# Nextomics/NextDenovo

Measured on AMD Instinct MI355X. Metric: corrected bases/sec, higher is better.
Workload: dtype int32

## Files before the change

### include/ndgpu_nextcorrect.h

```cpp
#ifndef NDGPU_NEXTCORRECT_H
#define NDGPU_NEXTCORRECT_H

#include <stdint.h>

#ifdef __cplusplus
extern "C" {
#endif
#pragma GCC visibility push(default)

typedef struct {
    unsigned int len;
    float identity;
    char *seq;
} consensus_trimed;

consensus_trimed *nextCorrect(char **seqs, unsigned int *aln_start, unsigned int *aln_end, unsigned int seq_count,
                              unsigned int max_mem_len, unsigned int min_len_aln, unsigned int max_cov_aln,
                              unsigned int min_cov, unsigned int lqseq_max_length, float min_error_corrected_ratio,
                              unsigned int split, unsigned int fast, int read_type);

void free_consensus_trimed(consensus_trimed *c);

typedef struct {
    unsigned int shift;
// ... 158 lines not shown
    uint64_t poa_resident_jobs;
    uint64_t poa_resident_declined;
    uint64_t poa_graph_launches;
    double poa_graph_ms;
    uint64_t poa_h2d_bytes;
    uint64_t poa_d2h_bytes;
    uint64_t cns_jobs;
    uint64_t cns_declined;
    uint64_t cns_launches;
    uint64_t cns_regions;
    double cns_ms;
    uint64_t cns_d2h_bytes;
    uint64_t walk_d2h_bytes;
} ndgpu_stats;
void ndgpu_get_stats(ndgpu_stats *out);
void ndgpu_reset_stats(void);
uint64_t ndgpu_release_memory(void);
void ndgpu_reserve_device_memory(uint64_t bytes);
int ndgpu_device_count(void);

#pragma GCC visibility pop
#ifdef __cplusplus
}
#endif
#endif
```

### nextdenovo_amd/api.py

```python
from __future__ import annotations

import ctypes as C
import os

os.environ.setdefault("GPU_MAX_HW_QUEUES", "16")

from . import build as _build

_LIB = None
_BIG = C.c_char * (1 << 30)


class ConsensusTrimed(C.Structure):
    _fields_ = [("len", C.c_uint), ("identity", C.c_float), ("seq", C.c_void_p)]


class PoaJob(C.Structure):
    _fields_ = [("seqs", C.POINTER(C.c_char_p)), ("len", C.POINTER(C.c_uint16)), ("seq_count", C.c_int32)]


class RankJob(C.Structure):
    _fields_ = [("seqs", C.POINTER(C.c_char_p)), ("len", C.POINTER(C.c_uint16)), ("seq_count", C.c_int32)]


# ... 100 lines not shown
    lib.ndgpu_poa_batch.argtypes = [C.POINTER(PoaJob), C.c_int, C.POINTER(C.c_void_p)]
    lib.ndgpu_poa_batch.restype = C.c_int
    lib.ndgpu_poa_batch_flags.argtypes = [C.POINTER(PoaJob), C.c_int, C.c_int, C.POINTER(C.c_void_p)]
    lib.ndgpu_poa_batch_flags.restype = C.c_int
    lib.ndgpu_lq_rank_batch.argtypes = [C.POINTER(RankJob), C.c_int, C.c_int, C.POINTER(RankResult)]
    lib.ndgpu_lq_rank_batch.restype = C.c_int
    lib.ndgpu_cns_windows_batch.argtypes = [C.POINTER(CnsJob), C.c_int, C.c_int, C.POINTER(CnsResult), C.POINTER(C.c_void_p),
                                            C.POINTER(C.c_void_p)]
    lib.ndgpu_cns_windows_batch.restype = C.c_int
    lib.ndgpu_align_batch.argtypes = [C.POINTER(AlnJob), C.c_int, C.c_int, C.POINTER(AlnResult), C.POINTER(C.c_void_p),
                                      C.POINTER(C.c_void_p), C.POINTER(C.c_void_p)]
    lib.ndgpu_align_batch.restype = C.c_int
    lib.ndgpu_align_db_batch.argtypes = [C.c_void_p, C.POINTER(AlnDbJob)] + lib.ndgpu_align_batch.argtypes[1:]
    lib.ndgpu_align_db_batch.restype = C.c_int
    lib.ndgpu_get_stats.argtypes = [C.POINTER(Stats)]
    lib.ndgpu_reset_stats.argtypes = []
    lib.ndgpu_device_count.restype = C.c_int
    return lib


def _take(lib, r):
    ln = r.contents.len
    ide = r.contents.identity
    seq = C.string_at(r.contents.seq, ln) if ln > 4 else b""
    lib.free_consensus_trimed(r)
    return ln, ide, seq


def correct(seqs, aln_start, aln_end, max_aln_length, min_len_aln=500, max_cov_aln=130, min_cov_base=4,
            max_lq_length=10000, min_error_corrected_ratio=0.8, split=0, fast=0, read_type=1):
# ... 328 lines not shown


def stats() -> dict:
    lib = load()
    s = Stats()
    lib.ndgpu_get_stats(C.byref(s))
    names = [f[0] for f in Stats._fields_]
    late = [n for n in names if n in _POA_RESIDENT_STATS]
    names = [n for n in names if n not in _POA_RESIDENT_STATS]
    at = names.index("poa_ms") + 1
    names[at:at] = late
    late = [n for n in names if n in _CNS_STATS]
    names = [n for n in names if n not in _CNS_STATS]
    at = names.index("backtrack_ms") + 1
    names[at:at] = late
    return {n: getattr(s, n) for n in names}


def release_device_memory() -> int:
    lib = load()
    lib.ndgpu_release_memory.restype = C.c_uint64
    return int(lib.ndgpu_release_memory())


def reserve_device_memory(n_bytes: int):
    lib = load()
    lib.ndgpu_reserve_device_memory.argtypes = [C.c_uint64]
    lib.ndgpu_reserve_device_memory.restype = None
    lib.ndgpu_reserve_device_memory(int(max(0, n_bytes)))


# ... 7 lines not shown
```

### nextdenovo_amd/csrc/capi.cpp

```cpp
#include <hip/hip_runtime_api.h>
#include <cerrno>
#include <sys/uio.h>
#include <unistd.h>

#include <algorithm>
#include <atomic>
#include <cstdio>
#include <cstdlib>
#include <cstring>
#include <string>
#include <chrono>
#include <functional>
#include <mutex>
#include <thread>
#include <vector>

#include "../../include/ndgpu_nextcorrect.h"
#include "nd_host.h"
#include "nd_cns.h"
#include "nd_runtime.h"
#include "nd_subplan.h"

using namespace ndgpu;

// ... 1011 lines not shown
    o->lq_aln_columns = s.lq_aln_columns, o->lq_bases = s.lq_bases, o->lq_out = s.lq_out;
    o->lq_jobs = s.lq_jobs, o->lq_repairs = s.lq_repairs;
    o->tb_tasks = s.tb_tasks, o->tb_walkers = s.tb_walkers, o->tb_fallbacks = s.tb_fallbacks;
    o->poa_jobs = s.poa_jobs, o->poa_declined = s.poa_declined, o->poa_rounds = s.poa_rounds, o->poa_launches = s.poa_launches;
    o->poa_cells = s.poa_cells, o->poa_ms = s.poa_ms;
    o->rank_jobs = s.rank_jobs, o->rank_tail = s.rank_tail, o->rank_launches = s.rank_launches, o->rank_ms = s.rank_ms;
    o->aln_batch_jobs = s.aln_batch_jobs, o->aln_batch_launches = s.aln_batch_launches, o->aln_batch_runs = s.aln_batch_runs;
    o->aln_batch_ms = s.aln_batch_ms;
    o->poa_resident_jobs = s.poa_resident_jobs, o->poa_resident_declined = s.poa_resident_declined;
    o->poa_graph_launches = s.poa_graph_launches, o->poa_graph_ms = s.poa_graph_ms;
    o->poa_h2d_bytes = s.poa_h2d_bytes, o->poa_d2h_bytes = s.poa_d2h_bytes;
    o->cns_jobs = s.cns_jobs, o->cns_declined = s.cns_declined, o->cns_launches = s.cns_launches, o->cns_regions = s.cns_regions;
    o->cns_ms = s.cns_ms, o->cns_d2h_bytes = s.cns_d2h_bytes, o->walk_d2h_bytes = s.walk_d2h_bytes;
}

void ndgpu_reset_stats(void) { DeviceAligner::reset_all_stats(); }

uint64_t ndgpu_release_memory(void) {
    size_t f0 = 0, f1 = 0, t = 0;
    (void)hipMemGetInfo(&f0, &t);
    join_reapers();
    for (int c = 0; c < DeviceAligner::kMaxContexts; c++)
        if (DeviceAligner *d = DeviceAligner::peek(c)) (void)d->release_memory_if_idle();
    (void)hipMemGetInfo(&f1, &t);
    return f1 > f0 ? (uint64_t)(f1 - f0) : 0;
}

void ndgpu_reserve_device_memory(uint64_t bytes) { DeviceAligner::reserve_device_memory(bytes); }

int ndgpu_device_count(void) {
// ... 7 lines not shown
```

### nextdenovo_amd/csrc/device_runtime.hip

```cpp
#include <hip/hip_runtime.h>

#include <algorithm>
#include <string>
#include <atomic>
#include <cassert>
#include <chrono>
#include <cmath>
#include <cstdio>
#include <cstdlib>
#include <cstring>
#include <condition_variable>
#include <mutex>
#include <set>
#include <thread>
#include <type_traits>
#include <unordered_map>
#include <vector>

#include "nd_device.h"
#include "nd_host.h"
#include "nd_lqplan.h"
#include "nd_runtime.h"

namespace ndgpu {
// ... 241 lines not shown
    X(uint32_t, d_ops, device, levelled)                                                                                                  \
    X(AlnTask, d_tasks, device, levelled)                                                                                                 \
    X(AlnOut, d_outs, device, levelled)                                                                                                   \
    X(uint64_t, d_trace, device, levelled)                                                                                                \
    X(int32_t, d_v, device, levelled)                                                                                                     \
                                                                  \
    X(uint64_t, d_wtrace, device, levelled)                                                                                               \
    X(int32_t, d_wmink, device, levelled)                                                                                                 \
    X(AlnTask, d_wtasks, device, levelled)        \
       \
    X(uint32_t, d_ck_cells, device, levelled)                                                                                             \
    X(uint2, d_ck_hdr, device, levelled)                                                                                                  \
    X(TbSeg, d_tbseg, device, levelled)                                                                                                   \
    X(TbSegOut, d_tbout, device, levelled)                                                                                                \
    X(int32_t, d_ids, device, levelled)                                                                                                   \
         \
    X(AlnRunSum, d_run_sums, device, levelled)                                                                                            \
    X(uint32_t, d_run_skip, device, levelled)                                                                                             \
    X(uint64_t, d_run_off, device, levelled)                                                                                              \
    X(uint32_t, d_runs, device, levelled)                                                                                                 \
                                                                                       \
    X(ReadDev, d_reads, device, levelled)                                                                                                 \
    X(PileDev, d_piles, device, levelled)                                                                                                 \
    X(uint32_t, d_read_pile, device, levelled)                                                                                            \
    X(uint32_t, d_acc, device, levelled)                                                                                                  \
    X(uint32_t, d_tags, device, levelled)                                                                                                 \
    X(uint32_t, d_colidx, device, levelled)                                                                                               \
    X(uint32_t, d_cov, device, levelled)                        \
    X(uint32_t, d_cellbase, device, levelled)                                                                                             \
    X(uint32_t, d_entbase, device, levelled)                                                                                              \
// ... 240 lines not shown
        if (dst_host && bytes) pending.push_back(Pending{dst_host, down_used, bytes});
        down_used += need;
        return at;
    }

    struct Phase {
        std::unique_lock<std::mutex> dbg;
        std::lock_guard<std::mutex> lock;
        explicit Phase(State &S) : dbg(g_debug_exclusive ? std::unique_lock<std::mutex>(g_dbg_mu) : std::unique_lock<std::mutex>()), lock(S.mu) {
            HIP_CHECK(hipSetDevice(S.device));
        }
    };

    std::vector<AlignChunk> plan_chunks(AlnTask *t, size_t nt);
    void launch_chunk(const AlignChunk &c, const int32_t *order, const int32_t *tb_order, hipEvent_t ev_mid, hipEvent_t ev_end, const char *who);
    void tally_outs(size_t nt, std::vector<int32_t> *wide);
    void run_wide(bool ops_to_host, const std::vector<int32_t> &ids);

    MainLayout layout_piles(MainPile **mp, size_t np);
    void reserve_layout(const MainLayout &L, size_t np);
    const int32_t *length_order(size_t a, size_t m);
    void align_main(const std::vector<AlignChunk> &chunks, size_t np);
    void launch_tags(const CovPlanes &cov, size_t np);
    void upload_plan(const MsaPlan &plan);
    MsaResult count_and_score(const MsaPlan &plan, const CovPlanes &cov, const CnsPlan *cns);
    CnsPlan plan_cns(const MsaPlan &plan, MainPile **mp);
    void launch_cns(const CnsPlan &cns, const PileDev *dev_piles, const PathItem *dev_path);
    void fetch_cns(const CnsPlan &cns, const MsaResult &res, const std::vector<uint8_t> &bad_pile, MainPile **mp);
    void score_pass(const MsaPlan &plan, const K10Args &k10);
    void rescue_pass(const MsaPlan &plan, const K10Args &k10);
// ... 118 lines not shown
        t.links += s.links; t.score_launches += s.score_launches; t.backtrack_ms += s.backtrack_ms;
        t.score_segments += s.score_segments; t.score_repairs += s.score_repairs; t.score_slow_piles += s.score_slow_piles;
        t.traceback_launches += s.traceback_launches; t.lq_launches += s.lq_launches; t.lq_columns += s.lq_columns;
        t.lq_aln_columns += s.lq_aln_columns; t.lq_bases += s.lq_bases; t.lq_out += s.lq_out; t.lq_jobs += s.lq_jobs; t.lq_repairs += s.lq_repairs;
        t.tb_tasks += s.tb_tasks; t.tb_walkers += s.tb_walkers; t.tb_fallbacks += s.tb_fallbacks;
        t.poa_jobs += s.poa_jobs; t.poa_declined += s.poa_declined; t.poa_rounds += s.poa_rounds; t.poa_launches += s.poa_launches;
        t.poa_cells += s.poa_cells; t.poa_ms += s.poa_ms;
        t.poa_resident_jobs += s.poa_resident_jobs; t.poa_resident_declined += s.poa_resident_declined;
        t.poa_graph_launches += s.poa_graph_launches; t.poa_graph_ms += s.poa_graph_ms;
        t.poa_h2d_bytes += s.poa_h2d_bytes; t.poa_d2h_bytes += s.poa_d2h_bytes;
        t.rank_jobs += s.rank_jobs; t.rank_tail += s.rank_tail; t.rank_launches += s.rank_launches; t.rank_ms += s.rank_ms;
        t.aln_batch_jobs += s.aln_batch_jobs; t.aln_batch_launches += s.aln_batch_launches; t.aln_batch_runs += s.aln_batch_runs;
        t.aln_batch_ms += s.aln_batch_ms;
        t.cns_jobs += s.cns_jobs; t.cns_declined += s.cns_declined; t.cns_launches += s.cns_launches; t.cns_regions += s.cns_regions;
        t.cns_ms += s.cns_ms; t.cns_d2h_bytes += s.cns_d2h_bytes; t.walk_d2h_bytes += s.walk_d2h_bytes;
    }
    t.allocs = g_alloc_calls.load(), t.alloc_ms = (double)g_alloc_ns.load() * 1e-6;
    t.level_allocs = g_level_calls.load(), t.level_ms = (double)g_level_ns.load() * 1e-6;
    return t;
}

void DeviceAligner::reset_all_stats() {
    g_alloc_calls = 0, g_alloc_ns = 0, g_level_calls = 0, g_level_ns = 0;
    for (int i = 0; i < kMaxContexts; i++)
        if (DeviceAligner *c = peek(i)) c->reset_stats();
}

uint32_t *DeviceAligner::upload_db(const uint32_t *pool_words, size_t n_words, int device) {
    HIP_CHECK(hipSetDevice(device));
    uint32_t *d = nullptr;
// ... 246 lines not shown
    if (max_sg) {
        d_ck_cells.reserve(max_ck * kCkptCells + 1);
        d_ck_hdr.reserve(max_ck + 1);
        d_tbseg.reserve(max_sg);
        d_tbout.reserve(max_sg);
    }
    return chunks;
}

void DeviceAligner::State::launch_chunk(const AlignChunk &c, const int32_t *order, const int32_t *tb_order, hipEvent_t ev_mid,
                                        hipEvent_t ev_end, const char *who) {
    const AlnTask *tk = d_tasks.p + c.begin;
    AlnOut *out = d_outs.p + c.begin;
    const int n = (int)(c.end - c.begin);
    const TbArgs tb{d_ck_cells.p, d_ck_hdr.p, d_tbseg.p, d_tbout.p, (int)c.slots, hooks_of<TbConfig>().cshift, hooks_of<TbConfig>().warm};
    if (c.seg) launch_ond_forward_ckpt(tk, out, d_pool.p, db_pool, d_trace.p, d_ops.p, tb, n, stream, order);
    else launch_ond_forward(tk, out, d_pool.p, db_pool, d_trace.p, n, stream, order);
    HIP_CHECK(hipEventRecord(ev_mid, stream));
    if (who) NDGPU_DBG(stream, "%s: traceback", who);
    if (c.seg) launch_ond_traceback_seg(tk, out, d_pool.p, db_pool, d_trace.p, d_ops.p, tb, n, stream);
    else launch_ond_traceback(tk, out, d_pool.p, db_pool, d_trace.p, nullptr, d_ops.p, nullptr, n, stream, tb_order);
    if (ev_end) HIP_CHECK(hipEventRecord(ev_end, stream));
}

void DeviceAligner::State::tally_outs(size_t nt, std::vector<int32_t> *wide) {
    for (size_t i = 0; i < nt; i++) {
        const AlnOut &o = h_outs.p[i];
        stats.cells += (uint64_t)o.cells;
        stats.d_steps += (uint64_t)o.d_steps;
        stats.trace_words += (uint64_t)o.trace_end;
        if (o.fin_idx & kTbSeen) {
            stats.tb_tasks++;
            stats.tb_walkers += (uint64_t)(o.d_final > 0 ? (o.d_final - 1) >> hooks_of<TbConfig>().cshift : 0) + 1;
            if (o.fin_idx & kTbRefused) stats.tb_fallbacks++;
        }
        if ((uint32_t)o.max_band > stats.max_band) stats.max_band = (uint32_t)o.max_band;
        if (wide && o.status == ST_NEED_WIDE) wide->push_back((int32_t)i);
        if (o.status == ST_ALIGNED) {
            stats.trace_bits += (uint64_t)o.cells;
            stats.columns += (uint64_t)o.n_cols;
        }
    }
}

static size_t next_chunk(AlnJob *const *jobs, size_t n, uint64_t trace_budget_bytes) {
    static const size_t max_jobs = getenv("NDGPU_ALIGN_CHUNK_JOBS") ? (size_t)std::max(1ll, atoll(getenv("NDGPU_ALIGN_CHUNK_JOBS"))) : ~(size_t)0;
    size_t take = 0;
    uint64_t bytes = 0;
    while (take < n && take < max_jobs) {
        const AlnJob &j = *jobs[take];
        int md, bd;
        limits_for(j.q_len + j.t_len, j.hq, &md, &bd);
        const uint64_t b = task_trace_bytes(md);
        if (take && bytes + b > trace_budget_bytes) break;
        bytes += b;
        take++;
    }
// ... 77 lines not shown
    pool.insert(pool.end(), kPoolPadWords, 0u);

    S.d_pool.reserve(pool.size());
    S.d_tasks.reserve(n);
    S.d_outs.reserve(n);
    const std::vector<AlignChunk> chunks = S.plan_chunks(tasks.data(), n);
    assert(chunks.size() == 1);
    S.d_ops.reserve(ops_words + 2);
    if (ops_to_host) S.h_ops.reserve(ops_words + 2);
    S.h_outs.reserve(n);

    hipStream_t st = S.stream;
    const uint64_t tc1 = wall_ns();
    S.h2d(S.d_pool.p, pool.data(), pool.size() * sizeof(uint32_t), st);
    S.h2d(S.d_tasks.p, tasks.data(), n * sizeof(AlnTask), st);
    S.mark(State::kEvFrontK7, st);
    NDGPU_DBG(st, "chunk: forward %zu tasks", n);
    S.launch_chunk(chunks[0], nullptr, nullptr, S.evs[State::kEvFrontK8a], nullptr, "chunk");
    NDGPU_DBG(st, "chunk: done");
    HIP_CHECK(hipMemcpyAsync(S.h_outs.p, S.d_outs.p, n * sizeof(AlnOut), hipMemcpyDeviceToHost, st));
    if (ops_to_host) HIP_CHECK(hipMemcpyAsync(S.h_ops.p, S.d_ops.p, ops_words * sizeof(uint32_t), hipMemcpyDeviceToHost, st));
    S.sync_drain(st);
    HIP_CHECK(hipGetLastError());
    S.stats.forward_ms += S.ms(State::kEvFrontK7, State::kEvFrontK8a);
    S.stats.forward_launches++;
    S.stats.tasks += n;

    std::vector<int32_t> wide;
    for (size_t i = 0; i < n; i++)
        if (S.h_outs.p[i].status == ST_NEED_WIDE) wide.push_back((int32_t)i);
    if (!wide.empty()) S.run_wide(ops_to_host, wide);
    *dev_ns = wall_ns() - tc1;

    S.tally_outs(n, nullptr);
    if (std::find(bad.begin(), bad.end(), 1) != bad.end()) {
        static bool warned = false;
// ... 261 lines not shown
    d_lq_jobs.reserve(L.jobs.size() + 1), d_lq_hdr.reserve(L.hdr_words + 1);
    d_lq_lnk.reserve(L.lnk_words + 64);
    d_lq_out.reserve(L.out_bytes + 1), d_lq_tmp.reserve(L.cell_rows + 1), d_lq_bnd.reserve((L.jobs.size() + 1) * 4 * (size_t)kLqLinkCap);
    return plan_chunks(tasks.data(), nt);
}

std::vector<char> DeviceAligner::State::launch_lq(LqLayout &L, const std::vector<AlignChunk> &chunks) {
    hipStream_t st = stream;
    const size_t n = L.piles.size(), nt = tasks.size();
    h2d(d_pool.p, pool.data(), pool.size() * sizeof(uint32_t), st);
    h2d(d_tasks.p, tasks.data(), nt * sizeof(AlnTask), st);
    h2d(d_lq_piles.p, L.piles.data(), n * sizeof(LqPileDev), st);
    h2d(d_lq_pieces.p, L.pieces.data(), L.pieces.size() * sizeof(LqPieceDev), st);
    if (!L.jobs.empty()) h2d(d_lq_jobs.p, L.jobs.data(), L.jobs.size() * sizeof(LqJobDev), st);
    grow_lq_evs(2 * chunks.size() + 1);
    HIP_CHECK(hipEventRecord(lq_evs[0], st));
    for (size_t c = 0; c < chunks.size(); c++) {
        NDGPU_DBG(st, "lq: forward / traceback %zu..%zu of %zu tasks", chunks[c].begin, chunks[c].end, nt);
        launch_chunk(chunks[c], nullptr, nullptr, lq_evs[2 * c + 1], lq_evs[2 * c + 2], nullptr);
    }
    mark(kEvLqMsaBegin, st);
    NDGPU_DBG(st, "lq: msa of %zu piles", n);
    launch_lq_msa(d_lq_piles.p, d_lq_jobs.p, d_lq_pieces.p, d_tasks.p, d_outs.p, d_ops.p, d_pool.p, d_lq_hdr.p, d_lq_lnk.p, d_lq_rec.p,
                  d_lq_bnd.p, d_lq_tmp.p, d_lq_out.p, (int)n, (int)L.jobs.size(), hooks_of<LqHooks>().warm, hooks_of<LqHooks>().force_repair, st);
    mark(kEvLqMsaEnd, st);
    h_outs.reserve(nt + 1);
    HIP_CHECK(hipMemcpyAsync(h_outs.p, d_outs.p, nt * sizeof(AlnOut), hipMemcpyDeviceToHost, st));
    std::vector<char> out(L.out_bytes + 1);
    d2h(L.piles.data(), d_lq_piles.p, n * sizeof(LqPileDev), st);
    if (L.out_bytes) d2h(out.data(), d_lq_out.p, L.out_bytes, st);
    sync_drain(st);
    HIP_CHECK(hipGetLastError());
    return out;
}

void DeviceAligner::State::tally_lq(LqRound **rounds, const LqLayout &L, size_t n_chunks, const std::vector<char> &out) {
    const size_t nt = tasks.size();
    for (size_t c = 0; c < n_chunks; c++) {
        stats.forward_ms += ms_between(lq_evs[2 * c], lq_evs[2 * c + 1]);
        stats.traceback_ms += ms_between(lq_evs[2 * c + 1], lq_evs[2 * c + 2]);
    }
    stats.forward_launches += n_chunks, stats.traceback_launches += n_chunks;
// ... 154 lines not shown
    auto cls_of = [&](size_t i) {
        const uint32_t c = ((uint32_t)tasks[a + i].q_len + (uint32_t)tasks[a + i].t_len) >> 6;
        return (kLenClasses - 1) - std::min<uint32_t>(c, kLenClasses - 1);
    };
    for (size_t i = 0; i < m; i++) order_cls[cls_of(i) + 1]++;
    for (uint32_t c = 0; c < kLenClasses; c++) order_cls[c + 1] += order_cls[c];
    for (size_t i = 0; i < m; i++) order[order_cls[cls_of(i)]++] = (int32_t)i;
    d_ids.reserve(m);
    h2d(d_ids.p, order.data(), m * sizeof(int32_t), stream);
    return d_ids.p;
}

void DeviceAligner::State::align_main(const std::vector<AlignChunk> &chunks, size_t np) {
    hipStream_t st = stream;
    const size_t nt = tasks.size();
    for (const AlignChunk &ch : chunks) {
        NDGPU_DBG(st, "main: forward %zu..%zu of %zu tasks, %zu piles", ch.begin, ch.end, nt, np);
        const int32_t *ids = length_order(ch.begin, ch.end - ch.begin);
        mark(kEvMainK7, st);
        launch_chunk(ch, ids, hooks_of<MainHooks>().k8_order ? ids : nullptr, evs[kEvMainK8a], evs[kEvMainAligned], "main");
        NDGPU_DBG(st, "main: traceback done");
        HIP_CHECK(hipEventSynchronize(evs[kEvMainAligned]));
        stats.forward_ms += ms(kEvMainK7, kEvMainK8a);
        stats.forward_launches++;
        stats.traceback_ms += ms(kEvMainK8a, kEvMainAligned);
        stats.traceback_launches++;
    }
    if (!nt) return;
    HIP_CHECK(hipMemcpyAsync(h_outs.p, d_outs.p, nt * sizeof(AlnOut), hipMemcpyDeviceToHost, st));
    sync_drain(st);
    std::vector<int32_t> wide;
    tally_outs(nt, &wide);
    if (!wide.empty()) run_wide(false, wide);
    stats.tasks += nt;
}

void DeviceAligner::State::launch_tags(const CovPlanes &cov, size_t np) {
    hipStream_t st = stream;
    const int nr = (int)reads.size();
    mark(kEvTagsBegin, st);
    NDGPU_DBG(st, "main: shift_scan");
    launch_shift_scan(d_tasks.p, d_outs.p, d_ops.p, d_reads.p, nr, st);
    NDGPU_DBG(st, "main: pile_accept");
    launch_pile_accept(d_piles.p, d_reads.p, d_acc.p, cov.cov, (int)np, st);
// ... 974 lines not shown
```

### nextdenovo_amd/csrc/nd_device.h

```cpp
#pragma once

#include <cstdint>

#include "nd_lockstep.h"

namespace ndgpu {

struct AlnTask {
    uint64_t q_off;
    uint64_t t_off;
    int32_t q_len;
    int32_t t_len;
    int32_t max_d;
    int32_t band;
    uint64_t trace_off;
    uint64_t mink_off;
    uint64_t ops_off;
    uint32_t ops_cap;
    uint32_t row_words;
    uint64_t v_off;
    uint32_t v_mask;
    uint32_t seg_off;
};

// ... 46 lines not shown
constexpr int32_t kTbRefused = 1 << 16;
constexpr int32_t kTbSeen = 1 << 17;

constexpr uint32_t kTagHead = 0u;
__host__ __device__ inline uint32_t tag_pack(int32_t t_pos, uint32_t delta, uint32_t base) {
    return ((uint32_t)(t_pos + 1) << 11) | (delta << 3) | base;
}
__host__ __device__ inline int32_t tag_tpos(uint32_t g) { return (int32_t)(g >> 11) - 1; }
__host__ __device__ inline uint32_t tag_delta(uint32_t g) { return (g >> 3) & 0xffu; }
__host__ __device__ inline uint32_t tag_base(uint32_t g) { return g & 7u; }

#if defined(SIMT_EMULATION)
inline unsigned long long wave_ballot(bool p) { return __ballot(p); }
#elif defined(__HIPCC__)
__device__ __forceinline__ unsigned long long wave_ballot(bool p) { return __builtin_amdgcn_ballot_w64(p); }
#endif

struct ReadDev {
    int32_t task;
    uint32_t aln_start;
    uint32_t aln_end;
    uint64_t tag_off;
    uint64_t colidx_off;
    uint32_t shift;
    uint32_t aln_len;
    uint32_t t_s, t_e;
    uint32_t q_start;
    uint32_t accepted;
    uint32_t pad_;
};
// ... 235 lines not shown
void launch_extract(const PileDev *piles, const ReadDev *reads, const uint32_t *acc_list, const uint32_t *tags,
                    const uint32_t *colidx, RegionDev *regions, char *strpool, unsigned long long *strpool_cursor,
                    unsigned long long strpool_cap, int n_regions, void *stream);

void launch_lq_rank(RegionDev *regions, const char *strpool, unsigned long long strpool_cap, uint32_t min_n, int n_regions, void *stream);

constexpr uint64_t kOffDb = 1ull << 63;
constexpr uint64_t kOffMask = kOffDb - 1;

constexpr uint32_t kPoolPadWords = 24;
constexpr uint32_t kTracePadWords = 16;
constexpr int kFastRowWords = 2;
constexpr int kFastMaxBand = 238;

void launch_ond_forward(const AlnTask *tasks, AlnOut *outs, const uint32_t *pool, const uint32_t *db_pool,
                        uint64_t *trace, int n_tasks, void *stream, const int32_t *order = nullptr);
struct TbArgs {
    uint32_t *ck_cells;
    void *ck_hdr;
    TbSeg *segs;
    TbSegOut *seg_outs;
    int n_slots;
    int cshift, warm;
};
void launch_ond_forward_ckpt(const AlnTask *tasks, AlnOut *outs, const uint32_t *pool, const uint32_t *db_pool, uint64_t *trace,
                             uint32_t *ops, const TbArgs &tb, int n_tasks, void *stream, const int32_t *order);
void launch_ond_traceback_seg(const AlnTask *tasks, AlnOut *outs, const uint32_t *pool, const uint32_t *db_pool, const uint64_t *trace,
                              uint32_t *ops, const TbArgs &tb, int n_tasks, void *stream);
void launch_ond_forward_wide(const AlnTask *tasks, AlnOut *outs, const uint32_t *pool, const uint32_t *db_pool,
                             uint64_t *trace, int32_t *trace_mink, int32_t *vscratch, const int32_t *task_ids, int n_ids, void *stream,
                             const AlnTask *wtasks = nullptr, uint32_t max_ring = 0);
constexpr size_t kWideLdsBytes = 64u << 10;
void launch_ond_traceback(const AlnTask *tasks, AlnOut *outs, const uint32_t *pool, const uint32_t *db_pool,
                          const uint64_t *trace,
                          const int32_t *trace_mink, uint32_t *ops, const int32_t *task_ids, int n, void *stream,
                          const int32_t *order = nullptr, const AlnTask *wtasks = nullptr);

struct AlnRunSum {
    uint32_t n_runs;
    uint32_t n_match, n_ins, n_del;
    uint32_t max_gap_run;
// ... 10 lines not shown
```

### nextdenovo_amd/csrc/nd_runtime.h

```cpp
#pragma once

#include <cstddef>
#include <cstdint>
#include <cstdlib>
#include <vector>

#include "nd_host.h"

namespace ndgpu {

struct RuntimeStats {
    uint64_t tasks = 0;
    uint64_t wide_tasks = 0;
    uint64_t cells = 0;
    uint64_t d_steps = 0;
    uint64_t trace_bits = 0;
    uint64_t columns = 0;
    uint64_t pool_bases = 0;
    uint64_t seq_bases = 0;
    uint32_t max_band = 0;
    uint32_t forward_launches = 0;
    double forward_ms = 0;
    double traceback_ms = 0;
    double tags_ms = 0;
// ... 44 lines not shown
    uint64_t aln_batch_runs = 0;
    double aln_batch_ms = 0;
    uint64_t poa_resident_jobs = 0;
    uint64_t poa_resident_declined = 0;
    uint64_t poa_graph_launches = 0;
    double poa_graph_ms = 0;
    uint64_t poa_h2d_bytes = 0;
    uint64_t poa_d2h_bytes = 0;
    uint64_t cns_jobs = 0;
    uint64_t cns_declined = 0;
    uint64_t cns_launches = 0;
    uint64_t cns_regions = 0;
    double cns_ms = 0;
    uint64_t cns_d2h_bytes = 0;
    uint64_t walk_d2h_bytes = 0;
};

struct CnsReq {
    const PathStep *steps = nullptr;
    size_t n = 0;
    int min_cov = 0;
    unsigned lq_max_len = 0;
    bool done = false;
    std::vector<uint32_t> words, wins;
    uint32_t counts[5] = {0, 0, 0, 0, 0};
};

struct DeviceOom {
    size_t bytes;
};
// ... 91 lines not shown
```

### nextdenovo_amd/csrc/ond_kernels.hip

```cpp
#include <hip/hip_runtime.h>

#include <climits>
#include <cstdlib>
#include <cstring>
#include <type_traits>

#include "nd_device.h"

namespace ndgpu {

namespace {

__device__ __forceinline__ int wave_max_i32(int v) {
    auto step = [](int x, auto ctrl, auto rows) {
        const int y = __builtin_amdgcn_update_dpp(INT_MIN, x, decltype(ctrl)::value, decltype(rows)::value, 0xf, false);
        return y > x ? y : x;
    };
    v = step(v, std::integral_constant<int, 0xb1>{}, std::integral_constant<int, 0xf>{});
    v = step(v, std::integral_constant<int, 0x4e>{}, std::integral_constant<int, 0xf>{});
    v = step(v, std::integral_constant<int, 0x141>{}, std::integral_constant<int, 0xf>{});
    v = step(v, std::integral_constant<int, 0x140>{}, std::integral_constant<int, 0xf>{});
    v = step(v, std::integral_constant<int, 0x142>{}, std::integral_constant<int, 0xa>{});
    v = step(v, std::integral_constant<int, 0x143>{}, std::integral_constant<int, 0xc>{});
    return __builtin_amdgcn_readlane(v, 63);
}

constexpr int kStreamBits = 56;
constexpr uint64_t kStreamMask = (1ull << kStreamBits) - 1;

__device__ __forceinline__ int wave_shr1(int first, int v) {
    return __builtin_amdgcn_update_dpp(first, v, 0x138, 0xf, 0xf, false);
}

struct Bases64 { uint32_t w[4]; };
static_assert(kPoolPadWords >= 5, "fetch64 reads five words from the word that holds a sequence's last base");
__device__ __forceinline__ Bases64 fetch64(const uint32_t *__restrict__ p, uint32_t sub);
__device__ __forceinline__ Bases64 fetch64_rel(const uint32_t *__restrict__ seq, uint32_t pos) { return fetch64(seq + (pos >> 4), pos & 15u); }
__device__ __forceinline__ Bases64 fetch64_abs(const uint32_t *__restrict__ pool, uint64_t off) {
    return fetch64(pool + (off >> 4), (uint32_t)(off & 15u));
}
__device__ __forceinline__ Bases64 fetch64(const uint32_t *__restrict__ p, uint32_t sub) {
    struct W4 { uint32_t x, y, z, w; } v;
    v.x = p[0], v.y = p[1], v.z = p[2], v.w = p[3];
    const uint32_t v4 = p[4];
    const uint32_t s = sub * 2u;
    Bases64 r;
    r.w[0] = __builtin_amdgcn_alignbit(v.y, v.x, s);
    r.w[1] = __builtin_amdgcn_alignbit(v.z, v.y, s);
    r.w[2] = __builtin_amdgcn_alignbit(v.w, v.z, s);
    r.w[3] = __builtin_amdgcn_alignbit(v4, v.w, s);
// ... 8 lines not shown
        const int rt = t_len - y;
        rem = rt < rem ? rt : rem;
        if (rem <= 0) break;
        const Bases64 a = fetch64_rel(qp, q_sh + (uint32_t)x);
        const Bases64 b = fetch64_rel(tp, t_sh + (uint32_t)y);
        const uint32_t d0 = a.w[0] ^ b.w[0], d1 = a.w[1] ^ b.w[1], d2 = a.w[2] ^ b.w[2], d3 = a.w[3] ^ b.w[3];
        int m = d0 ? (__builtin_ctz(d0) >> 1) : d1 ? 16 + (__builtin_ctz(d1) >> 1) : d2 ? 32 + (__builtin_ctz(d2) >> 1) : d3 ? 48 + (__builtin_ctz(d3) >> 1) : 64;
        m = m < rem ? m : rem;
        x += m;
        y += m;
        if (m < 64) break;
    }
    return x;
}

template <bool CKPT>
__global__ __launch_bounds__(64) void ond_forward_kernel(const AlnTask *__restrict__ tasks, AlnOut *__restrict__ outs,
                                                          const uint32_t *__restrict__ pool,
                                                          const uint32_t *__restrict__ db_pool,
                                                          uint64_t *__restrict__ trace, const int32_t *__restrict__ order,
                                                          uint32_t *__restrict__ ck_cells, uint2 *__restrict__ ck_hdr,
                                                          uint32_t *__restrict__ ops, int cshift) {
    const int tid = order ? order[blockIdx.x] : (int)blockIdx.x;
    const AlnTask T = tasks[tid];
    const int lane = (int)threadIdx.x;
    {
        const int total = T.q_len + T.t_len;
        if (total > 160000) __builtin_amdgcn_s_setprio(3);
        else if (total > 80000) __builtin_amdgcn_s_setprio(2);
        else if (total > 40000) __builtin_amdgcn_s_setprio(1);
    }

    int min_k = 0, max_k = 0, best_m = -1;
    int status = ST_NONE, fin_k = 0, fin_x = 0, fin_d = -1, fin_idx = 0;
    int d_steps = 0, max_band = 0;
    long long cells = 0;
    const int q_len = T.q_len, t_len = T.t_len;
    const uint64_t q_off = T.q_off & kOffMask, t_off = T.t_off & kOffMask;
    const uint32_t *__restrict__ qp = ((T.q_off >> 63) ? db_pool : pool) + (q_off >> 4);
    const uint32_t *__restrict__ tp = ((T.t_off >> 63) ? db_pool : pool) + (t_off >> 4);
    const uint32_t q_sh = (uint32_t)(q_off & 15u), t_sh = (uint32_t)(t_off & 15u);
    uint64_t *__restrict__ S = trace + T.trace_off;
    uint64_t rec = 0;
    uint32_t pos_base = 0, fill = 0;
    auto flush = [&]() {
        if ((uint32_t)lane < fill) S[pos_base + (uint32_t)lane] = rec;
        pos_base += fill;
        fill = 0;
    };
    auto put = [&](bool wide, uint64_t hi, uint64_t lo) {
        if (wide) {
            if ((uint32_t)lane == fill) rec = hi;
            fill++;
        }
        if ((uint32_t)lane == fill) rec = lo;
        fill++;
        if (fill >= 63u) flush();
    };
    if (CKPT) {
        uint32_t *__restrict__ W = ops + T.ops_off;
        const uint32_t nw = (T.ops_cap + 15u) / 16u + 1u;
        for (uint32_t i = (uint32_t)lane; i < nw; i += 64u) W[i] = 0u;
    }
    const int cmask = CKPT ? (1 << cshift) - 1 : 0;
    int porg0 = 0, porg1 = 0;
    int fin_org = 0;

    int px0 = 0, px1 = 0;
    int pj = 0;
    bool pwide = false;

    for (int d = 0; d < T.max_d && max_k - min_k <= T.band; d++) {
        const int band = max_k - min_k;
        if (band > kFastMaxBand) {
            status = ST_NEED_WIDE;
            break;
        }
        const int ncell = (band >> 1) + 1;
        const bool two = ncell > 64;
        d_steps++;
        cells += ncell;
        max_band = band > max_band ? band : max_band;

        const int src = pj + lane;
        int vp = __shfl(px0, src & 63, 64);
        int op = CKPT ? __shfl(porg0, src & 63, 64) : 0;
        if (pwide) {
            const int hi = __shfl(px1, src & 63, 64);
            vp = src >= 64 ? hi : vp;
            if (CKPT) {
                const int ohi = __shfl(porg1, src & 63, 64);
// ... 94 lines not shown
    flush();
    if (lane == 0) {
        AlnOut o;
        o.status = status;
        o.d_final = fin_d;
        o.k_final = fin_k;
        o.x_final = fin_x;
        o.y_final = fin_x - fin_k;
        o.n_cols = 0;
        o.d_steps = d_steps;
        o.max_band = max_band;
        o.cells = cells;
        o.trace_end = pos;
        o.fin_idx = fin_idx | (fin_org << 8);
        outs[tid] = o;
    }
}

constexpr int kWidePasses = 4;
template <bool LDSV>
__global__ __launch_bounds__(64) void ond_forward_wide_kernel(const AlnTask *__restrict__ tasks, AlnOut *__restrict__ outs,
                                                          const uint32_t *__restrict__ pool,
                                                          const uint32_t *__restrict__ db_pool,
                                                          uint64_t *__restrict__ trace,
                                                          int32_t *__restrict__ trace_mink,
                                                          int32_t *__restrict__ vscratch,
                                                          const int32_t *__restrict__ ids, const AlnTask *__restrict__ wtasks) {
    const int tid = ids[blockIdx.x];
    const AlnTask T = wtasks ? wtasks[blockIdx.x] : tasks[tid];
    const int lane = (int)threadIdx.x;
// ... 622 lines not shown

void launch_aln_runs_count(const AlnTask *tasks, const AlnOut *outs, const uint32_t *ops, const uint32_t *skip, AlnRunSum *sums, int n_tasks,
                           void *stream) {
    if (n_tasks <= 0) return;
    hipLaunchKernelGGL(aln_runs_kernel<false>, dim3((unsigned)n_tasks), dim3(64), 0, (hipStream_t)stream, tasks, outs, ops, skip, sums,
                       (const uint64_t *)nullptr, (uint32_t *)nullptr);
}

void launch_aln_runs_emit(const AlnTask *tasks, const AlnOut *outs, const uint32_t *ops, const AlnRunSum *sums, const uint64_t *run_off,
                          uint32_t *runs, int n_tasks, void *stream) {
    if (n_tasks <= 0) return;
    hipLaunchKernelGGL(aln_runs_kernel<true>, dim3((unsigned)n_tasks), dim3(64), 0, (hipStream_t)stream, tasks, outs, ops, (const uint32_t *)nullptr,
                       (AlnRunSum *)sums, run_off, runs);
}

void launch_ond_forward(const AlnTask *tasks, AlnOut *outs, const uint32_t *pool, const uint32_t *db_pool, uint64_t *trace,
                        int n_tasks, void *stream, const int32_t *order) {
    if (n_tasks <= 0) return;
    hipLaunchKernelGGL(ond_forward_kernel<false>, dim3((unsigned)n_tasks), dim3(64), 0, (hipStream_t)stream, tasks, outs, pool, db_pool, trace,
                       order, (uint32_t *)nullptr, (uint2 *)nullptr, (uint32_t *)nullptr, 0);
}

void launch_ond_forward_ckpt(const AlnTask *tasks, AlnOut *outs, const uint32_t *pool, const uint32_t *db_pool, uint64_t *trace,
                             uint32_t *ops, const TbArgs &tb, int n_tasks, void *stream, const int32_t *order) {
    if (n_tasks <= 0) return;
    static const size_t k7_lds = getenv("NDGPU_K7_LDS_KB") ? (size_t)atoi(getenv("NDGPU_K7_LDS_KB")) << 10 : 0;
    hipLaunchKernelGGL(ond_forward_kernel<true>, dim3((unsigned)n_tasks), dim3(64), k7_lds, (hipStream_t)stream, tasks, outs, pool, db_pool, trace,
                       order, tb.ck_cells, (uint2 *)tb.ck_hdr, ops, tb.cshift);
}

void launch_ond_traceback_seg(const AlnTask *tasks, AlnOut *outs, const uint32_t *pool, const uint32_t *db_pool, const uint64_t *trace,
                              uint32_t *ops, const TbArgs &tb, int n_tasks, void *stream) {
    if (n_tasks <= 0) return;
    const dim3 per_task((unsigned)((n_tasks + 63) / 64)), per_slot((unsigned)((tb.n_slots + 63) / 64));
    hipLaunchKernelGGL(tb_chase_kernel, per_task, dim3(64), 0, (hipStream_t)stream, tasks, outs, tb.ck_cells, (const uint2 *)tb.ck_hdr, tb.segs,
                       n_tasks, tb.cshift, tb.warm);
    static const size_t walk_lds = getenv("NDGPU_TB_LDS_KB") ? (size_t)atoi(getenv("NDGPU_TB_LDS_KB")) << 10 : 0;
    static const bool walk_win = !getenv("NDGPU_TB_WIN") || atoi(getenv("NDGPU_TB_WIN")) != 0;
    if (walk_win)
        hipLaunchKernelGGL(tb_walk_kernel<true>, per_slot, dim3(64), walk_lds, (hipStream_t)stream, tb.segs, tb.seg_outs, tasks, outs, pool, db_pool,
                           trace, ops, tb.n_slots);
    else
        hipLaunchKernelGGL(tb_walk_kernel<false>, per_slot, dim3(64), walk_lds, (hipStream_t)stream, tb.segs, tb.seg_outs, tasks, outs, pool, db_pool,
// ... 35 lines not shown
```

Before: 148.5 million.

## Add narrow-band fast path to O(ND) forward kernel with 64-base snake rounds

Adds a specialized inner loop in the forward alignment kernel for bands that fit in one wavefront (up to 110 diagonals). It uses 128-bit XOR and find-lowest-bit snake extension, cross-lane gathers and single-lane trace writes, and stays in a tight per-diagonal loop instead of the general path. The aim is to cut per-step overhead and ALU work in the common narrow-band case. It also adds per-task counters of narrow versus general steps, which cost an extra device buffer, D2H copy and host tally. The new path is on by default and can be turned off with an environment variable.

New measurement: 130.2 million. -12.4%, worse.

```diff
diff --git a/include/ndgpu_nextcorrect.h b/include/ndgpu_nextcorrect.h
--- a/include/ndgpu_nextcorrect.h
+++ b/include/ndgpu_nextcorrect.h
@@ -196,6 +196,7 @@
     uint64_t walk_d2h_bytes;
 } ndgpu_stats;
 void ndgpu_get_stats(ndgpu_stats *out);
+void ndgpu_get_k7_steps(uint64_t *narrow, uint64_t *general);
 void ndgpu_reset_stats(void);
 uint64_t ndgpu_release_memory(void);
 void ndgpu_reserve_device_memory(uint64_t bytes);
diff --git a/nextdenovo_amd/api.py b/nextdenovo_amd/api.py
--- a/nextdenovo_amd/api.py
+++ b/nextdenovo_amd/api.py
@@ -138,6 +138,8 @@
     lib.ndgpu_align_db_batch.argtypes = [C.c_void_p, C.POINTER(AlnDbJob)] + lib.ndgpu_align_batch.argtypes[1:]
     lib.ndgpu_align_db_batch.restype = C.c_int
     lib.ndgpu_get_stats.argtypes = [C.POINTER(Stats)]
+    lib.ndgpu_get_k7_steps.argtypes = [C.POINTER(C.c_uint64), C.POINTER(C.c_uint64)]
+    lib.ndgpu_get_k7_steps.restype = None
     lib.ndgpu_reset_stats.argtypes = []
     lib.ndgpu_device_count.restype = C.c_int
     return lib
@@ -496,7 +498,14 @@
     names = [n for n in names if n not in _CNS_STATS]
     at = names.index("backtrack_ms") + 1
     names[at:at] = late
-    return {n: getattr(s, n) for n in names}
+    out = {}
+    for n in names:
+        out[n] = getattr(s, n)
+        if n == "d_steps":
+            narrow, general = C.c_uint64(), C.c_uint64()
+            lib.ndgpu_get_k7_steps(C.byref(narrow), C.byref(general))
+            out["k7_steps_narrow"], out["k7_steps_general"] = int(narrow.value), int(general.value)
+    return out
 
 
 def release_device_memory() -> int:
diff --git a/nextdenovo_amd/csrc/capi.cpp b/nextdenovo_amd/csrc/capi.cpp
--- a/nextdenovo_amd/csrc/capi.cpp
+++ b/nextdenovo_amd/csrc/capi.cpp
@@ -1049,6 +1049,12 @@
     o->cns_ms = s.cns_ms, o->cns_d2h_bytes = s.cns_d2h_bytes, o->walk_d2h_bytes = s.walk_d2h_bytes;
 }
 
+void ndgpu_get_k7_steps(uint64_t *narrow, uint64_t *general) {
+    const RuntimeStats s = DeviceAligner::total_stats();
+    if (narrow) *narrow = s.k7_steps_narrow;
+    if (general) *general = s.k7_steps_general;
+}
+
 void ndgpu_reset_stats(void) { DeviceAligner::reset_all_stats(); }
 
 uint64_t ndgpu_release_memory(void) {
diff --git a/nextdenovo_amd/csrc/device_runtime.hip b/nextdenovo_amd/csrc/device_runtime.hip
--- a/nextdenovo_amd/csrc/device_runtime.hip
+++ b/nextdenovo_amd/csrc/device_runtime.hip
@@ -279,6 +279,7 @@
     X(TbSeg, d_tbseg, device, levelled)                                                                                                   \
     X(TbSegOut, d_tbout, device, levelled)                                                                                                \
     X(int32_t, d_ids, device, levelled)                                                                                                   \
+    X(uint32_t, d_k7narrow, device, levelled)                                     \
          \
     X(AlnRunSum, d_run_sums, device, levelled)                                                                                            \
     X(uint32_t, d_run_skip, device, levelled)                                                                                             \
@@ -549,6 +550,11 @@
 
     std::vector<AlignChunk> plan_chunks(AlnTask *t, size_t nt);
     void launch_chunk(const AlignChunk &c, const int32_t *order, const int32_t *tb_order, hipEvent_t ev_mid, hipEvent_t ev_end, const char *who);
+    std::vector<uint32_t> h_k7narrow;
+    void k7narrow_fetch(size_t nt, hipStream_t st) {
+        h_k7narrow.resize(nt);
+        d2h(h_k7narrow.data(), d_k7narrow.p, nt * sizeof(uint32_t), st);
+    }
     void tally_outs(size_t nt, std::vector<int32_t> *wide);
     void run_wide(bool ops_to_host, const std::vector<int32_t> &ids);
 
@@ -697,6 +703,7 @@
         t.aln_batch_ms += s.aln_batch_ms;
         t.cns_jobs += s.cns_jobs; t.cns_declined += s.cns_declined; t.cns_launches += s.cns_launches; t.cns_regions += s.cns_regions;
         t.cns_ms += s.cns_ms; t.cns_d2h_bytes += s.cns_d2h_bytes; t.walk_d2h_bytes += s.walk_d2h_bytes;
+        t.k7_steps_narrow += s.k7_steps_narrow; t.k7_steps_general += s.k7_steps_general;
     }
     t.allocs = g_alloc_calls.load(), t.alloc_ms = (double)g_alloc_ns.load() * 1e-6;
     t.level_allocs = g_level_calls.load(), t.level_ms = (double)g_level_ns.load() * 1e-6;
@@ -973,8 +980,9 @@
     AlnOut *out = d_outs.p + c.begin;
     const int n = (int)(c.end - c.begin);
     const TbArgs tb{d_ck_cells.p, d_ck_hdr.p, d_tbseg.p, d_tbout.p, (int)c.slots, hooks_of<TbConfig>().cshift, hooks_of<TbConfig>().warm};
-    if (c.seg) launch_ond_forward_ckpt(tk, out, d_pool.p, db_pool, d_trace.p, d_ops.p, tb, n, stream, order);
-    else launch_ond_forward(tk, out, d_pool.p, db_pool, d_trace.p, n, stream, order);
+    uint32_t *cnt = d_k7narrow.p + c.begin;
+    if (c.seg) launch_ond_forward_ckpt(tk, out, d_pool.p, db_pool, d_trace.p, d_ops.p, tb, n, stream, order, cnt);
+    else launch_ond_forward(tk, out, d_pool.p, db_pool, d_trace.p, n, stream, order, cnt);
     HIP_CHECK(hipEventRecord(ev_mid, stream));
     if (who) NDGPU_DBG(stream, "%s: traceback", who);
     if (c.seg) launch_ond_traceback_seg(tk, out, d_pool.p, db_pool, d_trace.p, d_ops.p, tb, n, stream);
@@ -983,10 +991,12 @@
 }
 
 void DeviceAligner::State::tally_outs(size_t nt, std::vector<int32_t> *wide) {
+    uint64_t narrow = 0, steps = 0;
     for (size_t i = 0; i < nt; i++) {
         const AlnOut &o = h_outs.p[i];
         stats.cells += (uint64_t)o.cells;
         stats.d_steps += (uint64_t)o.d_steps;
+        narrow += h_k7narrow[i], steps += (uint64_t)o.d_steps;
         stats.trace_words += (uint64_t)o.trace_end;
         if (o.fin_idx & kTbSeen) {
             stats.tb_tasks++;
@@ -1000,6 +1010,8 @@
             stats.columns += (uint64_t)o.n_cols;
         }
     }
+    stats.k7_steps_narrow += narrow, stats.k7_steps_general += steps - narrow;
+    if (trace_on()) fprintf(stderr, "[ndgpu trace] K7 steps: narrow %llu, general %llu\n", (unsigned long long)narrow, (unsigned long long)(steps - narrow));
 }
 
 static size_t next_chunk(AlnJob *const *jobs, size_t n, uint64_t trace_budget_bytes) {
@@ -1107,12 +1119,14 @@
     const uint64_t tc1 = wall_ns();
     S.h2d(S.d_pool.p, pool.data(), pool.size() * sizeof(uint32_t), st);
     S.h2d(S.d_tasks.p, tasks.data(), n * sizeof(AlnTask), st);
+    S.d_k7narrow.reserve(n);
     S.mark(State::kEvFrontK7, st);
     NDGPU_DBG(st, "chunk: forward %zu tasks", n);
     S.launch_chunk(chunks[0], nullptr, nullptr, S.evs[State::kEvFrontK8a], nullptr, "chunk");
     NDGPU_DBG(st, "chunk: done");
     HIP_CHECK(hipMemcpyAsync(S.h_outs.p, S.d_outs.p, n * sizeof(AlnOut), hipMemcpyDeviceToHost, st));
     if (ops_to_host) HIP_CHECK(hipMemcpyAsync(S.h_ops.p, S.d_ops.p, ops_words * sizeof(uint32_t), hipMemcpyDeviceToHost, st));
+    S.k7narrow_fetch(n, st);
     S.sync_drain(st);
     HIP_CHECK(hipGetLastError());
     S.stats.forward_ms += S.ms(State::kEvFrontK7, State::kEvFrontK8a);
@@ -1404,6 +1418,7 @@
     h2d(d_lq_pieces.p, L.pieces.data(), L.pieces.size() * sizeof(LqPieceDev), st);
     if (!L.jobs.empty()) h2d(d_lq_jobs.p, L.jobs.data(), L.jobs.size() * sizeof(LqJobDev), st);
     grow_lq_evs(2 * chunks.size() + 1);
+    d_k7narrow.reserve(nt);
     HIP_CHECK(hipEventRecord(lq_evs[0], st));
     for (size_t c = 0; c < chunks.size(); c++) {
         NDGPU_DBG(st, "lq: forward / traceback %zu..%zu of %zu tasks", chunks[c].begin, chunks[c].end, nt);
@@ -1416,6 +1431,7 @@
     mark(kEvLqMsaEnd, st);
     h_outs.reserve(nt + 1);
     HIP_CHECK(hipMemcpyAsync(h_outs.p, d_outs.p, nt * sizeof(AlnOut), hipMemcpyDeviceToHost, st));
+    k7narrow_fetch(nt, st);
     std::vector<char> out(L.out_bytes + 1);
     d2h(L.piles.data(), d_lq_piles.p, n * sizeof(LqPileDev), st);
     if (L.out_bytes) d2h(out.data(), d_lq_out.p, L.out_bytes, st);
@@ -1600,6 +1616,7 @@
 void DeviceAligner::State::align_main(const std::vector<AlignChunk> &chunks, size_t np) {
     hipStream_t st = stream;
     const size_t nt = tasks.size();
+    d_k7narrow.reserve(nt);
     for (const AlignChunk &ch : chunks) {
         NDGPU_DBG(st, "main: forward %zu..%zu of %zu tasks, %zu piles", ch.begin, ch.end, nt, np);
         const int32_t *ids = length_order(ch.begin, ch.end - ch.begin);
@@ -1614,6 +1631,7 @@
     }
     if (!nt) return;
     HIP_CHECK(hipMemcpyAsync(h_outs.p, d_outs.p, nt * sizeof(AlnOut), hipMemcpyDeviceToHost, st));
+    k7narrow_fetch(nt, st);
     sync_drain(st);
     std::vector<int32_t> wide;
     tally_outs(nt, &wide);
diff --git a/nextdenovo_amd/csrc/nd_device.h b/nextdenovo_amd/csrc/nd_device.h
--- a/nextdenovo_amd/csrc/nd_device.h
+++ b/nextdenovo_amd/csrc/nd_device.h
@@ -84,6 +84,36 @@
 inline unsigned long long wave_ballot(bool p) { return __ballot(p); }
 #elif defined(__HIPCC__)
 __device__ __forceinline__ unsigned long long wave_ballot(bool p) { return __builtin_amdgcn_ballot_w64(p); }
+#endif
+#if defined(SIMT_EMULATION)
+inline bool wave_lane_bit(unsigned long long m) { return (m >> (threadIdx.x & 63u)) & 1ull; }
+inline uint64_t wave_set_lane64(uint64_t old, uint32_t idx, uint64_t val) { return (threadIdx.x & 63u) == idx ? val : old; }
+inline int wave_gather(int v, int src) { return __shfl(v, src & 63, 64); }
+inline uint32_t lowest_bit(uint32_t v) { return v ? (uint32_t)__builtin_ctz(v) : 0xffffffffu; }
+inline int hide_value(int v) { return v; }
+#elif defined(__HIPCC__)
+__device__ __forceinline__ bool wave_lane_bit(unsigned long long m) { return __builtin_amdgcn_inverse_ballot_w64(m); }
+#pragma clang diagnostic push
+#pragma clang diagnostic ignored "-Winline-asm"
+__device__ __forceinline__ uint64_t wave_set_lane64(uint64_t old, uint32_t idx, uint64_t val) {
+    uint32_t lo = (uint32_t)old, hi = (uint32_t)(old >> 32);
+    asm("s_mov_b32 m0, %4\n\tv_writelane_b32 %0, %2, m0\n\tv_writelane_b32 %1, %3, m0"
+        : "+v"(lo), "+v"(hi)
+        : "s"((uint32_t)val), "s"((uint32_t)(val >> 32)), "s"(idx)
+        : "m0");
+    return (uint64_t)lo | ((uint64_t)hi << 32);
+}
+#pragma clang diagnostic pop
+__device__ __forceinline__ int wave_gather(int v, int src) { return __builtin_amdgcn_ds_bpermute((src << 2) & 0xfc, v); }
+__device__ __forceinline__ uint32_t lowest_bit(uint32_t v) {
+    uint32_t r;
+    asm("v_ffbl_b32 %0, %1" : "=v"(r) : "v"(v));
+    return r;
+}
+__device__ __forceinline__ int hide_value(int v) {
+    asm("" : "+v"(v));
+    return v;
+}
 #endif
 
 struct ReadDev {
@@ -349,7 +379,8 @@
 constexpr int kFastMaxBand = 238;
 
 void launch_ond_forward(const AlnTask *tasks, AlnOut *outs, const uint32_t *pool, const uint32_t *db_pool,
-                        uint64_t *trace, int n_tasks, void *stream, const int32_t *order = nullptr);
+                        uint64_t *trace, int n_tasks, void *stream, const int32_t *order = nullptr,
+                        uint32_t *narrow_steps = nullptr);
 struct TbArgs {
     uint32_t *ck_cells;
     void *ck_hdr;
@@ -359,7 +390,8 @@
     int cshift, warm;
 };
 void launch_ond_forward_ckpt(const AlnTask *tasks, AlnOut *outs, const uint32_t *pool, const uint32_t *db_pool, uint64_t *trace,
-                             uint32_t *ops, const TbArgs &tb, int n_tasks, void *stream, const int32_t *order);
+                             uint32_t *ops, const TbArgs &tb, int n_tasks, void *stream, const int32_t *order,
+                             uint32_t *narrow_steps = nullptr);
 void launch_ond_traceback_seg(const AlnTask *tasks, AlnOut *outs, const uint32_t *pool, const uint32_t *db_pool, const uint64_t *trace,
                               uint32_t *ops, const TbArgs &tb, int n_tasks, void *stream);
 void launch_ond_forward_wide(const AlnTask *tasks, AlnOut *outs, const uint32_t *pool, const uint32_t *db_pool,
diff --git a/nextdenovo_amd/csrc/nd_runtime.h b/nextdenovo_amd/csrc/nd_runtime.h
--- a/nextdenovo_amd/csrc/nd_runtime.h
+++ b/nextdenovo_amd/csrc/nd_runtime.h
@@ -82,6 +82,8 @@
     double cns_ms = 0;
     uint64_t cns_d2h_bytes = 0;
     uint64_t walk_d2h_bytes = 0;
+    uint64_t k7_steps_narrow = 0;
+    uint64_t k7_steps_general = 0;
 };
 
 struct CnsReq {
diff --git a/nextdenovo_amd/csrc/ond_kernels.hip b/nextdenovo_amd/csrc/ond_kernels.hip
--- a/nextdenovo_amd/csrc/ond_kernels.hip
+++ b/nextdenovo_amd/csrc/ond_kernels.hip
@@ -27,6 +27,7 @@
 
 constexpr int kStreamBits = 56;
 constexpr uint64_t kStreamMask = (1ull << kStreamBits) - 1;
+constexpr int kNarrowMaxBand = 2 * (kStreamBits - 1);
 
 __device__ __forceinline__ int wave_shr1(int first, int v) {
     return __builtin_amdgcn_update_dpp(first, v, 0x138, 0xf, 0xf, false);
@@ -34,6 +35,7 @@
 
 struct Bases64 { uint32_t w[4]; };
 static_assert(kPoolPadWords >= 5, "fetch64 reads five words from the word that holds a sequence's last base");
+static_assert(kPoolPadWords >= 6, "snake_round64 reads five words from the word that holds the base behind a sequence's last");
 __device__ __forceinline__ Bases64 fetch64(const uint32_t *__restrict__ p, uint32_t sub);
 __device__ __forceinline__ Bases64 fetch64_rel(const uint32_t *__restrict__ seq, uint32_t pos) { return fetch64(seq + (pos >> 4), pos & 15u); }
 __device__ __forceinline__ Bases64 fetch64_abs(const uint32_t *__restrict__ pool, uint64_t off) {
@@ -72,13 +74,31 @@
     return x;
 }
 
-template <bool CKPT>
+__device__ __forceinline__ int snake_round64(const uint32_t *__restrict__ qp, const uint32_t *__restrict__ tp, uint32_t q_sh, uint32_t t_sh,
+                                             int q_len, int t_len, int x, int y) {
+    const uint32_t qpos = q_sh + (uint32_t)(x < q_len ? x : q_len), tpos = t_sh + (uint32_t)(y < t_len ? y : t_len);
+    const Bases64 a = fetch64(qp + (qpos >> 4), qpos), b = fetch64(tp + (tpos >> 4), tpos);
+    const uint32_t u0 = lowest_bit(a.w[0] ^ b.w[0]), u1 = lowest_bit(a.w[1] ^ b.w[1]) | 32u, u2 = lowest_bit(a.w[2] ^ b.w[2]) | 64u,
+                   u3 = lowest_bit(a.w[3] ^ b.w[3]) | 96u;
+    uint32_t u = u0 < u1 ? u0 : u1;
+    u = u2 < u ? u2 : u;
+    u = u3 < u ? u3 : u;
+    u = u < 128u ? u : 128u;
+    int m = (int)(u >> 1);
+    const int rq = q_len - x, rt = t_len - y;
+    m = rq < m ? rq : m;
+    m = rt < m ? rt : m;
+    return m > 0 ? m : 0;
+}
+
+template <bool CKPT, bool NARROW>
 __global__ __launch_bounds__(64) void ond_forward_kernel(const AlnTask *__restrict__ tasks, AlnOut *__restrict__ outs,
                                                           const uint32_t *__restrict__ pool,
                                                           const uint32_t *__restrict__ db_pool,
                                                           uint64_t *__restrict__ trace, const int32_t *__restrict__ order,
                                                           uint32_t *__restrict__ ck_cells, uint2 *__restrict__ ck_hdr,
-                                                          uint32_t *__restrict__ ops, int cshift) {
+                                                          uint32_t *__restrict__ ops, int cshift,
+                                                          uint32_t *__restrict__ narrow_steps) {
     const int tid = order ? order[blockIdx.x] : (int)blockIdx.x;
     const AlnTask T = tasks[tid];
     const int lane = (int)threadIdx.x;
@@ -91,7 +111,7 @@
 
     int min_k = 0, max_k = 0, best_m = -1;
     int status = ST_NONE, fin_k = 0, fin_x = 0, fin_d = -1, fin_idx = 0;
-    int d_steps = 0, max_band = 0;
+    int d_steps = 0, max_band = 0, n_narrow = 0;
     long long cells = 0;
     const int q_len = T.q_len, t_len = T.t_len;
     const uint64_t q_off = T.q_off & kOffMask, t_off = T.t_off & kOffMask;
@@ -115,6 +135,11 @@
         fill++;
         if (fill >= 63u) flush();
     };
+    auto put_one = [&](uint64_t lo) {
+        rec = wave_set_lane64(rec, fill, lo);
+        fill++;
+        if (fill >= 63u) flush();
+    };
     if (CKPT) {
         uint32_t *__restrict__ W = ops + T.ops_off;
         const uint32_t nw = (T.ops_cap + 15u) / 16u + 1u;
@@ -133,6 +158,86 @@
         if (band > kFastMaxBand) {
             status = ST_NEED_WIDE;
             break;
+        }
+        if (NARROW && !pwide && band <= kNarrowMaxBand) {
+            const int d_in = d, nb_max = T.band < kNarrowMaxBand ? T.band : kNarrowMaxBand;
+            int to_ck = d ? -d & cmask : cmask + 1;
+            unsigned long long fb, leftm;
+            int x, org = 0;
+            unsigned int nc_sum = 0;
+            for (;;) {
+                const int nb = max_k - min_k, nc = (nb >> 1) + 1;
+                nc_sum += (unsigned int)nc;
+                max_band = nb > max_band ? nb : max_band;
+                const unsigned long long actm = (1ull << nc) - 1ull, topm = 1ull << (nc - 1);
+                const bool act = wave_lane_bit(actm);
+                const int src = pj + lane;
+                const int vp = wave_gather(px0, src);
+                const int vm = wave_shr1(0, vp);
+                const unsigned long long downm = (wave_ballot(vm < vp) & ~topm) | 1ull;
+                const bool down = wave_lane_bit(downm);
+                const int k0 = min_k + 2 * lane;
+                x = down ? vp : vm + 1;
+                if (CKPT) {
+                    const int op = wave_gather(porg0, src);
+                    const int om = wave_shr1(0, op);
+                    org = down ? op : om;
+                }
+                int m;
+                do {
+                    m = 0;
+                    if (act) {
+                        m = snake_round64(qp, tp, q_sh, t_sh, q_len, t_len, x, x - k0);
+                        x += m;
+                    }
+                    m = hide_value(m);
+                } while (wave_ballot(m == 64));
+                leftm = actm & ~downm;
+                fb = wave_ballot(x >= q_len) & wave_ballot(x - k0 >= t_len) & actm;
+                if (fb) break;
+                const int m2 = 2 * x - k0;
+                const int rb = wave_max_i32(act ? m2 : -1);
+                best_m = rb > best_m ? rb : best_m;
+                const unsigned long long okm = wave_ballot(m2 >= best_m - 150) & actm;
+                const unsigned long long qlo = okm & ~topm, qhi = okm & ~1ull;
+                const int j = qlo ? __builtin_ctzll(qlo) : nc - 1, jmax = qhi ? 63 - __builtin_clzll(qhi) : 0;
+                put_one(((uint64_t)j << (kStreamBits + 1)) | leftm);
+                x = act ? x : 0;
+                if (CKPT) {
+                    org = act ? org : 0;
+                    if (to_ck == 0) {
+                        to_ck = cmask + 1;
+                        const uint64_t slot = T.mink_off + (uint64_t)((d >> cshift) - 1);
+                        if (act) ck_cells[slot * kCkptCells + (uint32_t)lane] = (uint32_t)x | ((uint32_t)org << 24);
+                        if (lane == 0) ck_hdr[slot] = make_uint2(pos_base + fill, (uint32_t)min_k);
+                        org = lane;
+                    }
+                }
+                max_k = min_k + 2 * jmax + 1;
+                min_k = min_k + 2 * j - 1;
+                px0 = x;
+                porg0 = org;
+                pj = j;
+                to_ck--;
+                if ((d + 1 >= T.max_d) | (max_k - min_k > nb_max)) break;
+                d++;
+            }
+            d_steps += d - d_in + 1;
+            n_narrow += d - d_in + 1;
+            cells += nc_sum;
+            if (fb) {
+                fin_idx = __builtin_ctzll(fb);
+                fin_k = min_k + 2 * fin_idx;
+                fin_x = __builtin_amdgcn_readlane(x, fin_idx);
+                if (CKPT) fin_org = __builtin_amdgcn_readlane(org, fin_idx);
+                fin_d = d;
+                status = ST_FINISHED;
+                put_one(leftm);
+                break;
+            }
+            px1 = 0;
+            porg1 = CKPT && d && (d & cmask) == 0 ? 64 + lane : 0;
+            continue;
         }
         const int ncell = (band >> 1) + 1;
         const bool two = ncell > 64;
@@ -257,6 +362,7 @@
         o.trace_end = pos;
         o.fin_idx = fin_idx | (fin_org << 8);
         outs[tid] = o;
+        if (narrow_steps) narrow_steps[tid] = status != ST_NEED_WIDE ? (uint32_t)n_narrow : 0u;
     }
 }
 
@@ -909,19 +1015,33 @@
                        (AlnRunSum *)sums, run_off, runs);
 }
 
+static bool k7_narrow() {
+    static const bool on = !getenv("NDGPU_K7_NARROW") || atoi(getenv("NDGPU_K7_NARROW")) != 0;
+    return on;
+}
+
 void launch_ond_forward(const AlnTask *tasks, AlnOut *outs, const uint32_t *pool, const uint32_t *db_pool, uint64_t *trace,
-                        int n_tasks, void *stream, const int32_t *order) {
+                        int n_tasks, void *stream, const int32_t *order, uint32_t *narrow_steps) {
     if (n_tasks <= 0) return;
-    hipLaunchKernelGGL(ond_forward_kernel<false>, dim3((unsigned)n_tasks), dim3(64), 0, (hipStream_t)stream, tasks, outs, pool, db_pool, trace,
-                       order, (uint32_t *)nullptr, (uint2 *)nullptr, (uint32_t *)nullptr, 0);
+    if (k7_narrow())
+        hipLaunchKernelGGL((ond_forward_kernel<false, true>), dim3((unsigned)n_tasks), dim3(64), 0, (hipStream_t)stream, tasks, outs, pool, db_pool,
+                           trace, order, (uint32_t *)nullptr, (uint2 *)nullptr, (uint32_t *)nullptr, 0, narrow_steps);
+    else
+        hipLaunchKernelGGL((ond_forward_kernel<false, false>), dim3((unsigned)n_tasks), dim3(64), 0, (hipStream_t)stream, tasks, outs, pool, db_pool,
+                           trace, order, (uint32_t *)nullptr, (uint2 *)nullptr, (uint32_t *)nullptr, 0, narrow_steps);
 }
 
 void launch_ond_forward_ckpt(const AlnTask *tasks, AlnOut *outs, const uint32_t *pool, const uint32_t *db_pool, uint64_t *trace,
-                             uint32_t *ops, const TbArgs &tb, int n_tasks, void *stream, const int32_t *order) {
+                             uint32_t *ops, const TbArgs &tb, int n_tasks, void *stream, const int32_t *order,
+                             uint32_t *narrow_steps) {
     if (n_tasks <= 0) return;
     static const size_t k7_lds = getenv("NDGPU_K7_LDS_KB") ? (size_t)atoi(getenv("NDGPU_K7_LDS_KB")) << 10 : 0;
-    hipLaunchKernelGGL(ond_forward_kernel<true>, dim3((unsigned)n_tasks), dim3(64), k7_lds, (hipStream_t)stream, tasks, outs, pool, db_pool, trace,
-                       order, tb.ck_cells, (uint2 *)tb.ck_hdr, ops, tb.cshift);
+    if (k7_narrow())
+        hipLaunchKernelGGL((ond_forward_kernel<true, true>), dim3((unsigned)n_tasks), dim3(64), k7_lds, (hipStream_t)stream, tasks, outs, pool, db_pool,
+                           trace, order, tb.ck_cells, (uint2 *)tb.ck_hdr, ops, tb.cshift, narrow_steps);
+    else
+        hipLaunchKernelGGL((ond_forward_kernel<true, false>), dim3((unsigned)n_tasks), dim3(64), k7_lds, (hipStream_t)stream, tasks, outs, pool, db_pool,
+                           trace, order, tb.ck_cells, (uint2 *)tb.ck_hdr, ops, tb.cshift, narrow_steps);
 }
 
 void launch_ond_traceback_seg(const AlnTask *tasks, AlnOut *outs, const uint32_t *pool, const uint32_t *db_pool, const uint64_t *trace,
```
